# uingei/hevc

Hardware: AMD Instinct MI355X
Metric: encoded 1080p30 frames/sec/GPU; PSNR-Y parity vs libx265 at matched bitrate (higher is better)
Workload: dtype u8; 1 GPU; 1920x1080@30 SDR 8-bit Main, crf 19 capped by VBV maxrate 2940 kbps / bufsize 3528 kbit (the reference's libx265 operating point), 300-frame synthetic 'motion' clip per GPU, keyint 90 (4 closed GOPs of equal length), IPPP, full-search +-15, one clip per GPU, input resident in HBM

## Files before the change

### hevc_amd/_lib.py

```python
from __future__ import annotations

import ctypes as C
import numbers
import os
from pathlib import Path

HERE = Path(__file__).resolve().parent
LIB_PATH = Path(os.environ.get("MIHEVC_LIBRARY", HERE / "libmihevc.so"))

OK, EAGAIN, EOF, EINVAL, ENODEV, ENOMEM, EDEVICE, ESTATE = 0, -1, -2, -3, -4, -5, -6, -7


class Config(C.Structure):
    _fields_ = ([(n, C.c_int32) for n in (
        "width", "height", "fps_num", "fps_den", "bit_depth", "level_idc", "tier", "crf", "qp", "vbv_maxrate_kbps",
        "vbv_bufsize_kbits", "keyint", "min_keyint", "colour_primaries", "transfer", "matrix", "full_range", "chroma_loc",
        "aud", "repeat_headers", "hdr10")] +
        [("md_primaries", (C.c_uint16 * 2) * 3), ("md_white", C.c_uint16 * 2), ("md_max_lum", C.c_uint32), ("md_min_lum", C.c_uint32),
         ("max_cll", C.c_uint16), ("max_fall", C.c_uint16)] +
        [(n, C.c_int32) for n in ("me_range", "gops_in_flight", "host_threads", "sao", "profile_stages", "intra_tiles", "intra_nxn", "intra_in_p", "hrd", "pre_search", "rdo_zero", "chroma_modes", "pic_height", "slice_count", "slice_index")] +
        [("slice_ctu_rows", C.c_int32 * 16), ("rate_share_q16", C.c_int32), ("scenecut", C.c_int32), ("gop_balance", C.c_int32), ("rdo_cg", C.c_int32), ("p_tiles", C.c_int32), ("bframes", C.c_int32), ("b_qp_offset", C.c_int32), ("slice_halo", C.c_int32), ("slice_group", C.c_int32), ("sign_hide", C.c_int32), ("pic_hash", C.c_int32), ("ssim", C.c_int32)])


class Stats(C.Structure):
# ... 170 lines not shown
_PACKED_RGB = {"rgb": (0, 1, 2), "bgr": (2, 1, 0)}


def rgb_format_for(pix_fmt: str, matrix: int = 0, range: int = 0):
    import re
    name = (pix_fmt or "").lower()
    m = re.fullmatch(r"gbrp(?:(9|10|12|14|16)le|(f32le))?", name)
    if m:
        return RgbFormat(0, 2, 0, 1, 2 if m.group(2) else 0, 0 if m.group(2) else int(m.group(1) or 8), matrix, range)
    m = re.fullmatch(r"(rgb|bgr)(24|48le)", name)
    if m:
        return RgbFormat(3, *_PACKED_RGB[m.group(1)], 0, 8 if m.group(2) == "24" else 16, matrix, range)
    m = re.fullmatch(r"(rgb|bgr)(?:[a0]|(a64le))", name)
    if m:
        return RgbFormat(4, *_PACKED_RGB[m.group(1)], 0, 16 if m.group(2) else 8, matrix, range)
    m = re.fullmatch(r"[a0](rgb|bgr)", name)
    if m:
        return RgbFormat(4, *(i + 1 for i in _PACKED_RGB[m.group(1)]), 0, 8, matrix, range)
    return None


EXPORTS = (
    "mihevc_abi_version", "mihevc_device_count", "mihevc_device_numa_node", "mihevc_config_default", "mihevc_open", "mihevc_send_frame", "mihevc_send_frame_async", "mihevc_sync_uploads", "mihevc_send_frame_device", "mihevc_send_frames_device",
    "mihevc_receive_packet", "mihevc_flush", "mihevc_abort", "mihevc_close", "mihevc_get_stats", "mihevc_get_headers", "mihevc_set_keep_recon",
    "mihevc_get_recon", "mihevc_coded_size", "mihevc_get_frame_info", "mihevc_strerror", "mihevc_last_error", "mihevc_cost_params_for_qp", "mihevc_tile_grid", "mihevc_p_tile_grid", "mihevc_k_transform", "mihevc_k_transform_sdh",
    "mihevc_k_intra_frame", "mihevc_k_inter_frame", "mihevc_k_b_frame", "mihevc_k_deblock", "mihevc_k_sao", "mihevc_k_loop_filter", "mihevc_write_parameter_sets",
    "mihevc_encode_picture_host", "mihevc_k_picture_hash", "mihevc_write_picture_hash_sei", "mihevc_get_frame_quality", "mihevc_k_ssim",
    "mihevc_send_frame_fmt", "mihevc_k_convert_source", "mihevc_k_intra_plan", "mihevc_send_frame_rgb", "mihevc_k_convert_rgb",
    "mihevc_send_frame_scaled", "mihevc_k_scale_source", "mihevc_k_scene_diff", "mihevc_send_frame_deint", "mihevc_k_deinterlace",
    "mihevc_send_frame_denoise", "mihevc_k_denoise", "mihevc_send_frame_fieldmatch", "mihevc_get_fieldmatch_info", "mihevc_k_fieldmatch_metrics",
    "mihevc_k_fieldmatch_weave", "mihevc_set_lut3d", "mihevc_send_frame_lut3d", "mihevc_k_lut3d",
    "mihevc_send_frame_interpolate", "mihevc_k_mcfi_vectors", "mihevc_k_mcfi_render",
    "mihevc_send_frame_upscaled", "mihevc_k_upscale_source",
    "mihevc_set_sr_model", "mihevc_send_frame_sr", "mihevc_k_sr_conv", "mihevc_k_sr_input", "mihevc_k_sr_network",
)

_lib = None


class MihevcError(RuntimeError):
    def __init__(self, code: int, what: str = ""):
        self.code = code
        msg = strerror(code)
        super().__init__(f"{what}: {msg} ({code})" if what else f"{msg} ({code})")


def load() -> C.CDLL:
    global _lib
    if _lib is not None:
        return _lib
    if not LIB_PATH.exists():
        raise OSError(f"{LIB_PATH} not built: run `python -c 'import __graft_entry__ as g; g.build()'` (hipcc --offload-arch=gfx950)")
    lib = C.CDLL(str(LIB_PATH))
    for name in EXPORTS:
        getattr(lib, name)
    vp, i32, i64 = C.c_void_p, C.c_int, C.c_int64
    lib.mihevc_strerror.restype = C.c_char_p
    lib.mihevc_last_error.restype = C.c_char_p
    lib.mihevc_last_error.argtypes = [vp]
    lib.mihevc_config_default.argtypes = [C.POINTER(Config)]
    lib.mihevc_config_default.restype = None
    lib.mihevc_open.argtypes = [C.POINTER(Config), i32, C.POINTER(vp)]
    lib.mihevc_send_frame.argtypes = [vp, vp, vp, vp, i32, i32, i64]
    lib.mihevc_send_frame_device.argtypes = [vp, vp, vp, vp, i32, i32, i64]
    lib.mihevc_send_frame_async.argtypes = [vp, vp, vp, vp, i32, i32, i64]
    lib.mihevc_send_frames_device.argtypes = [vp, i32, vp, vp, vp, i32, i32, i64]
    lib.mihevc_sync_uploads.argtypes = [vp]
    lib.mihevc_receive_packet.argtypes = [vp, C.POINTER(C.POINTER(C.c_uint8)), C.POINTER(C.c_size_t), C.POINTER(i64), C.POINTER(i64), C.POINTER(i32)]
    lib.mihevc_flush.argtypes = [vp]
    lib.mihevc_abort.argtypes = [vp]
    lib.mihevc_close.argtypes = [vp]
    lib.mihevc_close.restype = None
    lib.mihevc_get_stats.argtypes = [vp, C.POINTER(Stats)]
    lib.mihevc_get_headers.argtypes = [vp, C.POINTER(C.POINTER(C.c_uint8)), C.POINTER(C.c_size_t)]
    lib.mihevc_set_keep_recon.argtypes = [vp, i32]
    lib.mihevc_get_recon.argtypes = [vp, i64, vp, vp, vp]
    lib.mihevc_coded_size.argtypes = [vp, C.POINTER(i32), C.POINTER(i32)]
    lib.mihevc_get_frame_info.argtypes = [vp, i64, C.POINTER(i32), C.POINTER(i32), C.POINTER(i64)]
    lib.mihevc_cost_params_for_qp.argtypes = [i32, i32, i32, C.POINTER(CostParams)]
    lib.mihevc_cost_params_for_qp.restype = None
    lib.mihevc_k_transform.argtypes = [i32, vp, vp, vp, i32, i32, i32, i32, i32, i32]
    lib.mihevc_k_transform_sdh.argtypes = [i32, vp, vp, vp, i32, i32, i32, i32, i32, i32, i32, i32]
    lib.mihevc_k_intra_frame.argtypes = [i32, vp, vp, vp, i32, i32, C.POINTER(CostParams), vp, vp, vp, vp, vp, vp, vp, vp]
    lib.mihevc_k_intra_plan.argtypes = [i32, vp, vp, vp, i32, i32, C.POINTER(CostParams), vp]
    lib.mihevc_k_inter_frame.argtypes = [i32, vp, vp, vp, vp, vp, vp, i32, i32, C.POINTER(CostParams), vp, vp, vp, vp, vp, vp, vp, vp, vp, vp]
    lib.mihevc_k_b_frame.argtypes = [i32] + [vp] * 9 + [i32, i32, C.POINTER(CostParams)] + [vp] * 12
    lib.mihevc_k_deblock.argtypes = [i32, vp, vp, vp, i32, i32, vp, i32]
    lib.mihevc_k_sao.argtypes = [i32, vp, vp, vp, vp, vp, vp, i32, i32, C.POINTER(CostParams), vp, vp, vp, vp]
    lib.mihevc_k_loop_filter.argtypes = [i32, vp, vp, vp, vp, vp, vp, i32, i32, vp, C.POINTER(CostParams), vp, vp, vp, vp]
    lib.mihevc_write_parameter_sets.argtypes = [C.POINTER(Config), vp, C.c_size_t]
    lib.mihevc_encode_picture_host.argtypes = [C.POINTER(Config), i32, i32, i32, vp, vp, vp, vp, vp, vp, C.c_size_t]
# ... 70 lines not shown
```

### hevc_amd/csrc/bitstream.cpp

```cpp
#include "bitstream.h"

#include <algorithm>
#include <cstdlib>
#include <cstring>

namespace mihevc {

void BitWriter::put(uint32_t v, int n)
{
    while (n > 0) {
        int take = std::min(n, 8 - nbits_);
        uint32_t chunk = (n == 32 && take == 32) ? v : ((v >> (n - take)) & ((1u << take) - 1));
        acc_ = (acc_ << take) | chunk;
        nbits_ += take;
        n -= take;
        if (nbits_ == 8) {
            buf_.push_back((uint8_t)acc_);
            acc_ = 0;
            nbits_ = 0;
        }
    }
}
void BitWriter::ue(uint32_t v)
{
// ... 623 lines not shown
    const TileGrid &grid() const { return grid_; }
    const std::string &error() const { return err_; }
    size_t run_tile(int tx, int ty, std::vector<uint8_t> &out)
    {
        cabac_.redirect(out);
        cabac_.init(pic_.slice_type, pic_.qp);
        const bool last_tile = tx == grid_.cols - 1 && ty == grid_.rows - 1;
        const int x1 = grid_.col_bd(tx + 1), y1 = grid_.row_bd(ty + 1);
        for (int ry = grid_.row_bd(ty); ry < y1; ry++)
            for (int rx = grid_.col_bd(tx); rx < x1; rx++) {
                if (pic_.sao) sao(rx, ry);
                quadtree(rx << kCtuLog2, ry << kCtuLog2, kCtuLog2, 0);
                cabac_.terminate(last_tile && ry == y1 - 1 && rx == x1 - 1);
            }
        if (!last_tile) cabac_.terminate(1);
        cabac_.finish();
        return cabac_.bins();
    }

private:
    const mihevc_cu_rec &cu(int x, int y) const { return pic_.cu[(y >> 3) * w8_ + (x >> 3)]; }
    static int zorder6(int bx, int by)
    {
        int z = 0;
        for (int i = 0; i < 3; i++) z |= ((bx >> i) & 1) << (2 * i) | ((by >> i) & 1) << (2 * i + 1);
        return z;
    }
    int zaddr(int x, int y) const { return (((y >> kCtuLog2) * wc_ + (x >> kCtuLog2)) << 6) | zorder6((x & 31) >> 2, (y & 31) >> 2); }
    bool avail(int xc, int yc, int xn, int yn) const
    {
        if (!(xn >= 0 && yn >= 0 && xn < w_ && yn < h_ && zaddr(xn, yn) <= zaddr(xc, yc))) return false;
        return !grid_.on() || (grid_.col_of(xn >> kCtuLog2) == grid_.col_of(xc >> kCtuLog2) && grid_.row_of(yn >> kCtuLog2) == grid_.row_of(yc >> kCtuLog2));
    }

    void sao(int rx, int ry)
    {
        const mihevc_sao_ctu &s = pic_.sao[ry * wc_ + rx];
        auto same = [](const mihevc_sao_ctu &a, const mihevc_sao_ctu &b) {
            if (a.type[0] != b.type[0] || a.type[1] != b.type[1]) return false;
            for (int c = 0; c < 3; c++) {
                int t = a.type[c ? 1 : 0];
                if (!t) continue;
                if (memcmp(a.offset[c], b.offset[c], 4)) return false;
                if (t == 1 && a.band_pos[c] != b.band_pos[c]) return false;
                if (t == 2 && c < 2 && a.eo_class[c] != b.eo_class[c]) return false;
            }
            return true;
        };
        if (rx > grid_.col_bd(grid_.col_of(rx))) {
// ... 343 lines not shown
                cabac_.bin(kCsbf + ((right | below) ? 1 : 0) + (c_idx ? 2 : 0), 0);
                continue;
            }
            int lev[16], nsig = 0, first_sig = 16, last_sig = -1, abs_sum = 0;
            int start = i == last_sb ? last_pos : 15;
            for (int k = 0; k < 16; k++) {
                lev[k] = k <= start ? b[pscan[k][1] * stride + pscan[k][0]] : 0;
                if (lev[k]) { nsig++; first_sig = std::min(first_sig, k); last_sig = k; abs_sum += std::abs(lev[k]); }
            }
            const bool hidden = sdh && last_sig - first_sig > 3;
            if (hidden && (abs_sum & 1) != (lev[first_sig] < 0) && err_.empty()) {
                const int sh = c_idx ? 1 : 0;
                err_ = "sign data hiding: CTU (" + std::to_string((tu_x << sh) >> kCtuLog2) + ", " + std::to_string((tu_y << sh) >> kCtuLog2) + ") plane " +
                       std::to_string(c_idx) + ": the 4x4 group at (" + std::to_string(tu_x + 4 * xs) + ", " + std::to_string(tu_y + 4 * ys) +
                       ") has an absolute sum whose parity does not match its first level's sign";
            }
            bool infer_dc = false;
            if (i < last_sb && i > 0) {
                csbf[ys][xs] = nsig != 0;
                cabac_.bin(kCsbf + ((right | below) ? 1 : 0) + (c_idx ? 2 : 0), nsig != 0);
                infer_dc = true;
            } else csbf[ys][xs] = 1;
            if (!csbf[ys][xs]) continue;
            int prev = right + 2 * below;
            for (int k = (i == last_sb ? last_pos - 1 : 15); k >= 0; k--) {
                if (k == 0 && infer_dc) break;
                int xp = pscan[k][0], yp = pscan[k][1], xc = (xs << 2) + xp, yc = (ys << 2) + yp, sc;
                if (log2n == 2) { static const uint8_t m[16] = {0, 1, 4, 5, 2, 3, 4, 5, 6, 6, 8, 8, 7, 7, 8, 8}; sc = m[(yc << 2) + xc]; }
                else if (xc + yc == 0) sc = 0;
                else {
                    if (prev == 0) sc = (xp + yp == 0) ? 2 : (xp + yp < 3) ? 1 : 0;
                    else if (prev == 1) sc = yp == 0 ? 2 : yp == 1 ? 1 : 0;
                    else if (prev == 2) sc = xp == 0 ? 2 : xp == 1 ? 1 : 0;
                    else sc = 2;
                    if (c_idx == 0) { if (xs || ys) sc += 3; sc += log2n == 3 ? (scan == 0 ? 9 : 15) : 21; }
                    else sc += log2n == 3 ? 9 : 12;
                }
                cabac_.bin(kSig + (c_idx ? 27 + sc : sc), lev[k] != 0);
                if (lev[k]) infer_dc = false;
            }
            if (!nsig) continue;
            int ctx_set = (i > 0 && c_idx == 0) ? 2 : 0;
            if (c1_carry == 0) ctx_set++;
            int c1 = 1, ng1 = 0, g2_pos = -1;
            for (int k = 15; k >= 0; k--) {
                if (!lev[k]) continue;
                if (ng1 == 8) break;
                int g1 = std::abs(lev[k]) > 1;
                cabac_.bin(kG1 + ctx_set * 4 + c1 + (c_idx ? 16 : 0), g1);
                ng1++;
                if (g1) { c1 = 0; if (g2_pos < 0) g2_pos = k; }
                else if (c1 > 0 && c1 < 3) c1++;
            }
            c1_carry = c1;
            if (g2_pos >= 0) cabac_.bin(kG2 + ctx_set + (c_idx ? 4 : 0), std::abs(lev[g2_pos]) > 2);
            uint32_t signs = 0; int ns = 0;
            for (int k = 15; k >= 0; k--) if (lev[k]) { signs = (signs << 1) | (uint32_t)(lev[k] < 0); ns++; }
            if (hidden) { signs >>= 1; ns--; }
            cabac_.bypass_bits(signs, ns);
            int num = 0, rice = 0;
            for (int k = 15; k >= 0; k--) {
                if (!lev[k]) continue;
                int a = std::abs(lev[k]);
                int base = num < 8 ? (k == g2_pos ? 3 : 2) : 1;
                if (a >= base) {
                    remaining(a - base, rice);
                    if (a > 3 * (1 << rice)) rice = std::min(rice + 1, 4);
                }
                num++;
            }
        }
    }
    void remaining(int v, int rice)
    {
        int q = v >> rice;
        if (q < 4) {
            for (int i = 0; i < q; i++) cabac_.bypass(1);
            cabac_.bypass(0);
            cabac_.bypass_bits((uint32_t)(v & ((1 << rice) - 1)), rice);
        } else {
            for (int i = 0; i < 4; i++) cabac_.bypass(1);
            int k = rice + 1, r = v - (4 << rice);
            while (r >= (1 << k)) { cabac_.bypass(1); r -= 1 << k; k++; }
            cabac_.bypass(0);
            cabac_.bypass_bits((uint32_t)r, k);
        }
    }

    const mihevc_config &cfg_;
    const PictureSyms &pic_;
    std::vector<uint8_t> scratch_;
    Cabac cabac_;
// ... 108 lines not shown
```

### hevc_amd/csrc/session.cpp

```cpp
#include <algorithm>
#include <chrono>
#include <cstdlib>
#include <cstring>
#include <numeric>
#include <thread>

#include "md5.h"
#include "session.h"

constexpr int kSeamRows = 8;

int fail(mihevc_session *s, std::string msg)
{
    { std::lock_guard<std::mutex> l(s->m); s->err = std::move(msg); }
    s->failed = true;
    if (s->group) s->group->fail();
    return MIHEVC_EDEVICE;
}

int alloc_planes(mihevc_session *s, CachedBlock<uint8_t> mem[3], void *p[3], int stride[3], int padded)
{
    for (int i = 0; i < 3; i++) {
        int w = i ? s->w / 2 : s->w, h = i ? s->h / 2 : s->h, pad = padded == 1 ? (i ? PAD_C : PAD_Y) : 0, vm = padded == 2 ? (i ? kSeamRows / 2 : kSeamRows) : pad;
        stride[i] = (w + 2 * pad + 63) & ~63;
// ... 563 lines not shown

template <typename T> std::vector<FrameRec> lane_records(mihevc_session *s, const Chunk<T> &c, int g, int upto)
{
    std::vector<FrameRec> v((size_t)upto);
    std::lock_guard<std::mutex> l(s->m);
    for (int j = 0; j < upto; j++) v[(size_t)j] = s->frames[c.fidx(g, j)];
    return v;
}

int slice_sums(mihevc_session *s, const std::vector<size_t> &idx, bool with_est)
{
    const size_t n = idx.size();
    std::vector<double> v(with_est ? 2 * n : n);
    {
        std::lock_guard<std::mutex> l(s->m);
        for (size_t i = 0; i < n; i++) { v[i] = (double)s->frames[idx[i]].bits_local; if (with_est) v[n + i] = (double)s->frames[idx[i]].est_local; }
    }
    if (int e = group_sum(s, v)) return e;
    std::lock_guard<std::mutex> l(s->m);
    for (size_t i = 0; i < n; i++) { auto &fr = s->frames[idx[i]]; fr.bits = (long long)v[i]; if (with_est) { fr.est_q4 = (unsigned long long)v[n + i]; fr.est_known = true; } }
    return 0;
}

int lane_estimates(mihevc_session *s, const SymLayout &sl, int slot, const std::vector<int> &lanes, std::vector<unsigned long long> &out)
{
    std::vector<double> v(lanes.size(), 0.0);
    for (size_t k = 0; k < lanes.size(); k++) {
        unsigned long long e = 0;
        HIPCK(s, hipMemcpy(&e, s->lane[lanes[k]].sym_dev[slot] + sl.est, sizeof e, hipMemcpyDeviceToHost));
        v[k] = (double)e;
    }
    if (int e = group_sum(s, v)) return e;
    out.assign(v.begin(), v.end());
    return 0;
}
std::vector<int> first_lanes(int n) { std::vector<int> v((size_t)n); std::iota(v.begin(), v.end(), 0); return v; }

int mark(mihevc_session *s, hipStream_t st, int stage, int pictures, bool begin)
{
    if (!s->cfg.profile_stages || (s->cfg.profile_stages == 2 && stage != 2)) return 0;
    size_t need_ev = s->marks.size() * 2 + 2;
    while (s->ev_pool.size() < need_ev) { s->ev_pool.emplace_back(hipEventDefault); if (!s->ev_pool.back()) return fail(s, "hipEventCreate failed"); }
    if (begin) { s->marks.push_back({stage, pictures, s->marks.size() * 2}); HIPCK(s, hipEventRecord(s->ev_pool[s->marks.back().ev], st)); }
    else HIPCK(s, hipEventRecord(s->ev_pool[s->marks.back().ev + 1], st));
    return 0;
}
#define STAGE(st, idx, pics, call) do { if (int e_ = mark(s, st, idx, pics, true)) return e_; HIPCK(s, call); if (int e_ = mark(s, st, idx, pics, false)) return e_; } while (0)

template <typename T> int rate_feedback(mihevc_session *s, const Chunk<T> &c, const Part &p, int t)
{
    const int p_slots = s->ring - 1;
    if (c.halo.on && s->rc.rc_on && t - p_slots >= 1) {
        std::vector<size_t> idx;
        for (int g = 0; g < c.gl.batch[(size_t)(t - p_slots)]; g++) idx.push_back(c.fidx(g, t - p_slots));
        if (int e = slice_sums(s, idx, false)) return e;
    }
    if (t >= 2) HIPCK(s, hipStreamWaitEvent(p.st, s->slot[t == 2 ? 0 : p.grp][c.slot_of(t - 2)].copy, 0));
    if (!s->rc.rc_on || t < 3) return 0;
    const int j = t - 2;
    const Part pj = c.part(s, p.grp, j);
    HIPCK(s, hipEventSynchronize(s->slot[p.grp][c.slot_of(j)].copy));
    std::vector<double> v((size_t)pj.n);
    for (int k = 0; k < pj.n; k++) v[(size_t)k] = (double)*(const unsigned long long *)(s->lane[pj.lanes[(size_t)k]].sym_host[c.slot_of(j)] + c.sl.est);
    if (int e = group_sum(s, v)) return e;
    std::lock_guard<std::mutex> l(s->m);
    for (int k = 0; k < pj.n; k++) { auto &fr = s->frames[c.fidx(pj.lanes[(size_t)k], j)]; if (!fr.est_known) { fr.est_q4 = (unsigned long long)v[(size_t)k]; fr.est_known = true; } }
    return 0;
}

template <typename T> int rho_trial(mihevc_session *s, const Chunk<T> &c, const std::vector<int> &want, const std::vector<unsigned long long> &ev, const std::vector<int> &qa)
{
    const int B1 = c.gl.batch[1], tb = c.steps;
    memcpy(c.ha + (size_t)tb * c.lay.total, c.ha + (size_t)1 * c.lay.total, c.lay.total);
    StepView<T> tv(c.ha, c.lay, tb), dtv(c.da, c.lay, tb), h0(c.ha, c.lay, 0), h1(c.ha, c.lay, 1);
    std::vector<int> qp_trial((size_t)B1);
    for (int g = 0; g < B1; g++) {
        mihevc_session::Lane &L = s->lane[g];
        const int a = c.at(1, g);
        qp_trial[(size_t)g] = RateControl::trial_qp(want[(size_t)g]);
        tv.sao[a] = h0.sao[c.at(0, g)];
        tv.sao[a].sao = nullptr; tv.sao[a].sse = nullptr; tv.sao[a].sse_ctu = nullptr; tv.sao[a].cu = nullptr;
        tv.sao[a].halo_top = tv.sao[a].halo_bottom = 0;
        tv.inter[a] = h1.inter[a];
        for (int i = 0; i < 3; i++) tv.inter[a].rec[i] = mk<T>(L.rec_p[1][i], L.rec_stride[i]);
        tv.inter[a].prm = prm_for(s, qp_trial[(size_t)g]);
        tv.inter[a].ip = nullptr;
        HIPCK(s, hipMemsetAsync(L.sym_dev[c.slot_of(1)] + c.sl.sse, 0, 4 * sizeof(unsigned long long), s->st_compute));
    }
    HIPCK(s, hipMemcpyAsync(c.da + (size_t)tb * c.lay.total, c.ha + (size_t)tb * c.lay.total, c.lay.total, hipMemcpyHostToDevice, s->st_compute));
    HIPCK(s, launch_sao<T>(s->st_compute, dtv.sao, s->w, s->h, B1, false));
    HIPCK(s, launch_pad<T>(s->st_compute, dtv.sao, s->w, s->h, B1));
    if (s->cfg.pre_search) HIPCK(s, hipStreamWaitEvent(s->st_compute, s->ev_pre, 0));
    HIPCK(s, launch_me_search<T>(s->st_compute, dtv.inter, s->n_ctu, B1, s->me_range));
    HIPCK(s, launch_inter_ctu<T>(s->st_compute, dtv.inter, s->n_ctu, B1, s->me_range));
    HIPCK(s, hipStreamSynchronize(s->st_compute));
    std::vector<unsigned long long> ep;
    if (int e = lane_estimates(s, c.sl, c.slot_of(1), first_lanes(B1), ep)) return e;
    s->rc.measure_rho(ep, qp_trial, ev, qa);
    return 0;
}

template <typename T> int idr_step(mihevc_session *s, const Chunk<T> &c, std::vector<int> &qp_step)
{
    const int B = c.gl.batch[0];
    StepView<T> dv(c.da, c.lay, 0), hv(c.ha, c.lay, 0);
    HIPCK(s, hipMemcpyAsync(c.da, c.ha, c.lay.total, hipMemcpyHostToDevice, s->st_compute));
    for (int g = 0; g < B; g++) HIPCK(s, hipMemsetAsync(s->lane[g].sym_dev[0] + c.sl.sse, 0, 4 * sizeof(unsigned long long), s->st_compute));
    STAGE(s->st_compute, 0, B, launch_intra_picture<T>(s->st_compute, dv.intra, s->ctus_w, s->ctus_h, B, s->tiles.cols, s->tiles.rows, s->cfg.pre_search ? s->ev_args : nullptr));
    if (s->cfg.pre_search) {
        HIPCK(s, hipStreamWaitEvent(s->st_pre, s->ev_args, 0));
        HIPCK(s, launch_pre_search_chunk<T>(s->st_pre, (const PreArgs<T> *)(c.da + c.flat_off), s->w, s->h, s->n_ctu, c.n_pre));
        HIPCK(s, hipEventRecord(s->ev_pre, s->st_pre));
    }
    if (!s->rc.rc_on) return 0;
    HIPCK(s, hipStreamSynchronize(s->st_compute));
    std::vector<unsigned long long> ev, e2;
    if (int e = lane_estimates(s, c.sl, 0, first_lanes(B), ev)) return e;
    const std::vector<int> qa(qp_step);
    std::vector<int> want((size_t)B);
    for (int g = 0; g < B; g++) want[(size_t)g] = s->rc.want_idr(g, ev[(size_t)g], qa[(size_t)g]);
    if (!s->rc.rho_measured && c.steps > 1 && c.gl.batch[1] > 0) {
        if (int e = rho_trial<T>(s, c, want, ev, qa)) return e;
        for (int g = 0; g < B; g++) want[(size_t)g] = s->rc.want_idr(g, ev[(size_t)g], qa[(size_t)g]);
    }
    std::vector<int> redo;
    for (int g = 0; g < B; g++)
        if (RateControl::redo_idr(want[(size_t)g], qa[(size_t)g])) redo.push_back(g);
    if (!redo.empty()) {
        for (size_t k = 0; k < redo.size(); k++) {
            const int g = redo[k];
            qp_step[(size_t)g] = want[(size_t)g];
            patch_qp<T>(s, c, 0, g, qp_step[(size_t)g]);
            hv.intra[B + (int)k] = hv.intra[c.at(0, g)];
            HIPCK(s, hipMemsetAsync(s->lane[g].sym_dev[0] + c.sl.sse, 0, 4 * sizeof(unsigned long long), s->st_compute));
        }
        HIPCK(s, hipMemcpyAsync(c.da, c.ha, c.lay.total, hipMemcpyHostToDevice, s->st_compute));
        STAGE(s->st_compute, 0, (int)redo.size(), launch_intra_picture<T>(s->st_compute, dv.intra + B, s->ctus_w, s->ctus_h, (int)redo.size(), s->tiles.cols, s->tiles.rows, nullptr));
        HIPCK(s, hipStreamSynchronize(s->st_compute));
        if (int e = lane_estimates(s, c.sl, 0, redo, e2)) return e;
        for (size_t k = 0; k < redo.size(); k++) ev[(size_t)redo[k]] = e2[k];
    }
    s->rc.idr_settled(qp_step);
    std::lock_guard<std::mutex> l(s->m);
    for (int g = 0; g < B; g++) { auto &fr = s->frames[c.fidx(g, 0)]; fr.est_q4 = ev[(size_t)g]; fr.est_known = true; }
    return 0;
}

template <typename T> int inter_step(mihevc_session *s, const Chunk<T> &c, const Part &p, int t)
{
    const int B = p.n;
    hipStream_t st = p.st;
    StepView<T> dv(c.da, c.lay, t, p.base), hv(c.ha, c.lay, t, p.base), pv(c.da, c.lay, t - 1, c.group_base(p.grp, t - 1));
    StepParams sp{};
    sp.p_tile_cols = s->ptiles.cols; sp.p_tile_rows = s->ptiles.rows;
    for (int g = 0; g < B; g++) sp.prm[g] = hv.inter[g].prm;
    if (c.halo.on && c.halo.reach > 0) {
        if (int e = wait_neighbours(s, c.halo, 2, s->gstep + t - 1)) return e;
        HIPCK(s, launch_copy_rows(st, c.halo.jobs(t, c.halo.jl.pull), B * 3 * c.halo.reach, 16));
    }
    HIPCK(s, launch_prep_p_step<T>(st, pv.sao, (const PreArgs<T> *)nullptr, dv.intra, dv.inter, dv.sao, sp, s->w, s->h, B));
    if (t == 1 && s->cfg.pre_search) HIPCK(s, hipStreamWaitEvent(st, s->ev_pre, 0));
    const bool bstep = type_of_step(c.bf, t) == 0;
// ... 329 lines not shown
{
    if (!s) return MIHEVC_EINVAL;
    if (s->failed) return s->fail_code;
    if (s->flushed) return MIHEVC_OK;
    if (int e = source_flush(s)) return e;
    s->flushing = true;
    int e = run_chunk(s);
    s->flushed = true;
    return e;
}

int mihevc_abort(mihevc_session *s)
{
    if (!s) return MIHEVC_EINVAL;
    { std::lock_guard<std::mutex> l(s->m); if (s->err.empty()) s->err = "aborted by the caller"; }
    s->failed = true;
    if (s->group) s->group->fail();
    return MIHEVC_OK;
}

int mihevc_receive_packet(mihevc_session *s, const uint8_t **data, size_t *size, int64_t *pts, int64_t *dts, int *keyframe)
{
    if (!s || !data || !size) return MIHEVC_EINVAL;
    std::unique_lock<std::mutex> l(s->m);
    auto it = s->packets.find(s->next_out);
    if (it == s->packets.end() || !it->second.ready) return (s->flushed && s->next_out >= s->frames_in) ? MIHEVC_EOF : MIHEVC_EAGAIN;
    if (!it->second.error.empty()) { std::string err = it->second.error; l.unlock(); s->fail_code = MIHEVC_EINVAL; fail(s, err); return MIHEVC_EINVAL; }
    s->cur_packet = std::move(it->second.data);
    if (pts) *pts = it->second.pts;
    if (dts) *dts = it->second.dts;
    if (keyframe) *keyframe = it->second.key;
    s->packets.erase(it);
    s->next_out++;
    s->stats.frames_out = s->next_out;
    *data = s->cur_packet.data();
    *size = s->cur_packet.size();
    return MIHEVC_OK;
}

int mihevc_get_headers(mihevc_session *s, const uint8_t **data, size_t *size)
{
    if (!s || !data || !size) return MIHEVC_EINVAL;
    *data = s->headers.data();
    *size = s->headers.size();
    return MIHEVC_OK;
}

int mihevc_get_stats(const mihevc_session *s, mihevc_stats *out)
{
    if (!s || !out) return MIHEVC_EINVAL;
    std::lock_guard<std::mutex> l(const_cast<mihevc_session *>(s)->m);
    *out = s->stats;
    out->entropy_ms = (double)s->entropy_ns.load() / 1e6;
    double *ssim[3] = {&out->ssim_y, &out->ssim_u, &out->ssim_v};
    for (int c = 0; c < 3; c++) *ssim[c] = s->cfg.ssim ? (double)s->ssim_total[c] / ((double)ssim_window_count(s, c) * 4294967296.0) : 0.0;
    return MIHEVC_OK;
}

int mihevc_set_keep_recon(mihevc_session *s, int keep)
{
    if (!s) return MIHEVC_EINVAL;
    s->keep_recon = keep != 0;
// ... 66 lines not shown
```

### hevc_amd/csrc/session.h

```cpp
#pragma once
#include <hip/hip_runtime.h>

#include <atomic>
#include <condition_variable>
#include <map>
#include <mutex>
#include <string>
#include <vector>

#include "bitstream.h"
#include "device.h"
#include "gop_plan.h"
#include "host_pool.h"
#include "ratectl.h"
#include "scale_taps.h"
#include "slice_group.h"

using namespace mihevc;

constexpr int kRing = 12;
constexpr int kGroups = 2;

struct Packet {
    std::vector<uint8_t> data;
// ... 42 lines not shown
    int keyint = 90, lanes = 4, me_range = 16, qp_p = 22, qp_i = 19;
    bool is16 = false, keep_recon = false, flushed = false, flushing = false;
    std::atomic<bool> failed{false};
    int fail_code = MIHEVC_EDEVICE;
    std::string err;
    CachedStream st_compute, st_copy, st_pre;
    int lane_groups = kGroups;
    Event ev_up{hipEventDisableTiming};
    bool up_pending = false;
    std::vector<Src> pending;
    std::vector<Src> free_src;
    SourceFront src;
    struct Lane {
        CachedBlock<uint8_t> rec_mem[3][3]; void *rec_p[3][3] = {}; int rec_stride[3] = {};
        CachedBlock<uint8_t> work_mem[3]; void *work_p[3] = {}; int work_stride[3] = {};
        CachedBlock<int32_t> me, me1;
        CachedBlock<IpInfo> ip;
        CachedBlock<IntraPlan> plan;
        CachedBlock<uint8_t> sym_dev[kRing], sym_host[kRing];
        CachedBlock<uint8_t> md5_host[kRing];
    };
    std::vector<Lane> lane;
    CachedBuf args;
    struct Slot { Event compute{hipEventDisableTiming}, copy{hipEventDisableTiming}; int jobs_open = 0; } slot[kGroups][kRing];
    Event ev_join{hipEventDisableTiming};
    Event t_begin{hipEventDefault}, t_end{hipEventDefault};
    std::vector<Event> ev_pool;
    struct Mark { int stage, pictures; size_t ev; };
    std::vector<Mark> marks;
    ThreadPool *pool = nullptr;
    std::mutex m;
    std::condition_variable cv;
    int ring = 8;
    int host_threads = 2;
    std::map<int64_t, Packet> packets;
    int64_t next_out = 0, frames_in = 0, frames_done = 0;
    std::vector<uint8_t> headers, cur_packet;
    std::map<int64_t, std::vector<uint16_t>> recon;
    mihevc_stats stats{};
    RateControl rc;
    CachedBuf probe;
    int64_t pts_step = 1, first_pts = 0;
    GopState gop;
    CachedBuf low;
    Event ev_pre{hipEventDisableTiming}, ev_args{hipEventDisableTiming};
    CachedBuf scene;
    std::vector<FrameRec> frames;
    struct Quality { unsigned long long sse[3]; long long ssim[3]; bool known; };
    std::vector<Quality> quality;
    std::atomic<long long> entropy_ns{0};
    bool events_ok() const
    {
        bool ok = ev_up && ev_join && t_begin && t_end && ev_pre && ev_args;
        for (auto &g : slot) for (auto &sl : g) ok = ok && sl.compute && sl.copy;
        return ok;
    }
    std::shared_ptr<SliceGroup> group;
    int band = 0, n_bands = 1;
    int band_h[kMaxBands] = {0};
    long long gstep = 0;
// ... 21 lines not shown
```

### hevc_amd/encoder.py

```python
from __future__ import annotations

import ctypes as C
import logging
import re
import threading
from fractions import Fraction
from pathlib import Path
from typing import Callable, Iterator, Optional, Tuple

import numpy as np

from . import _lib
from .probe import VideoInfo

logger = logging.getLogger(__name__)

_COLOUR_CODES = {
    "primaries": {"bt709": 1, "bt470bg": 5, "smpte170m": 6, "bt2020": 9},
    "transfer": {"bt709": 1, "smpte170m": 6, "smpte2084": 16, "pq": 16, "arib-std-b67": 18, "bt2020-10": 14},
    "matrix": {"bt709": 1, "bt470bg": 5, "smpte170m": 6, "bt2020nc": 9, "bt2020-ncl": 9, "bt2020": 9},
}


_DEPTH_IN_FMT = re.compile(r'(?:p|gray|gbrp|yuva?\d{3}p?)(9|10|12|14|16)(?:le|be)?$|^(?:p0|p2|p4|y2)(10|12|16)(?:le|be)?$')
# ... 38 lines not shown
            cfg.md_primaries[i][0], cfg.md_primaries[i][1] = x, y
        cfg.md_white[0], cfg.md_white[1] = md.wp
        cfg.md_max_lum, cfg.md_min_lum = md.lum
        cfg.max_cll, cfg.max_fall = parse_max_cll(max_cll or info.max_cll)
    else:
        cfg.colour_primaries = _COLOUR_CODES["primaries"].get(info.color_primaries, 1)
        cfg.transfer = _COLOUR_CODES["transfer"].get(info.color_transfer, 1)
        cfg.matrix = _COLOUR_CODES["matrix"].get(info.color_space, 1)
    return cfg


class Encoder:

    def __init__(self, cfg: _lib.Config, device: int = 0, keep_recon: bool = False):
        self._lib = _lib.load()
        self.cfg = cfg
        self._s = C.c_void_p()
        rc = self._lib.mihevc_open(C.byref(cfg), device, C.byref(self._s))
        if rc != 0:
            raise _lib.MihevcError(rc, "mihevc_open")
        if keep_recon:
            self._lib.mihevc_set_keep_recon(self._s, 1)
        self._pts = 0

    def close(self):
        if self._s:
            self._lib.mihevc_close(self._s)
            self._s = C.c_void_p()

    def __enter__(self):
        return self

    def __exit__(self, *exc):
        self.close()

    def _check(self, rc, what):
        if rc != 0:
            detail = self._lib.mihevc_last_error(self._s).decode() if self._s else ""
            raise _lib.MihevcError(rc, f"{what} {detail}".strip())

    def send(self, y: np.ndarray, u: np.ndarray, v: np.ndarray, pts: Optional[int] = None):
        c = self.cfg
        dt = np.uint8 if c.bit_depth == 8 else np.uint16
        if y.shape != (c.height, c.width) or u.shape != (c.height // 2, c.width // 2) or v.shape != u.shape:
            raise ValueError(f"plane shapes {y.shape}/{u.shape}/{v.shape} do not match the session's {c.width}x{c.height} 4:2:0")
        for p in (y, u, v):
# ... 249 lines not shown

    def sync_uploads(self):
        self._check(self._lib.mihevc_sync_uploads(self._s), "sync_uploads")

    def send_device(self, y_ptr: int, u_ptr: int, v_ptr: int, pitch_y: int, pitch_c: int, pts: Optional[int] = None):
        pts = self._pts if pts is None else pts
        self._pts = pts + 1
        self._check(self._lib.mihevc_send_frame_device(self._s, y_ptr, u_ptr, v_ptr, pitch_y, pitch_c, pts), "send_frame_device")

    def send_device_batch(self, y_ptrs, u_ptrs, v_ptrs, pitch_y: int, pitch_c: int, first_pts: Optional[int] = None):
        n = len(y_ptrs)
        arrs = [p if isinstance(p, C.Array) else (C.c_void_p * n)(*p) for p in (y_ptrs, u_ptrs, v_ptrs)]
        pts = self._pts if first_pts is None else first_pts
        self._pts = pts + n
        self._check(self._lib.mihevc_send_frames_device(self._s, n, arrs[0], arrs[1], arrs[2], pitch_y, pitch_c, pts), "send_frames_device")

    def flush(self):
        self._check(self._lib.mihevc_flush(self._s), "flush")

    def abort(self):
        if self._s:
            self._lib.mihevc_abort(self._s)

    def packets(self) -> Iterator[Tuple[bytes, int, bool]]:
        data, size = C.POINTER(C.c_uint8)(), C.c_size_t()
        pts, dts, key = C.c_int64(), C.c_int64(), C.c_int()
        while True:
            rc = self._lib.mihevc_receive_packet(self._s, C.byref(data), C.byref(size), C.byref(pts), C.byref(dts), C.byref(key))
            if rc in (_lib.EAGAIN, _lib.EOF):
                return
            self._check(rc, "receive_packet")
            yield C.string_at(data, size.value), pts.value, bool(key.value)

    def packets_dts(self) -> Iterator[Tuple[bytes, int, bool, int]]:
        data, size = C.POINTER(C.c_uint8)(), C.c_size_t()
        pts, dts, key = C.c_int64(), C.c_int64(), C.c_int()
        while True:
            rc = self._lib.mihevc_receive_packet(self._s, C.byref(data), C.byref(size), C.byref(pts), C.byref(dts), C.byref(key))
            if rc in (_lib.EAGAIN, _lib.EOF):
                return
            self._check(rc, "receive_packet")
            yield C.string_at(data, size.value), pts.value, bool(key.value), dts.value

    def headers(self) -> bytes:
        data, size = C.POINTER(C.c_uint8)(), C.c_size_t()
        self._check(self._lib.mihevc_get_headers(self._s, C.byref(data), C.byref(size)), "get_headers")
        return C.string_at(data, size.value)

    def stats(self) -> _lib.Stats:
        st = _lib.Stats()
        self._check(self._lib.mihevc_get_stats(self._s, C.byref(st)), "get_stats")
        return st

    def coded_size(self) -> Tuple[int, int]:
        w, h = C.c_int(), C.c_int()
        self._lib.mihevc_coded_size(self._s, C.byref(w), C.byref(h))
        return w.value, h.value

    def recon(self, index: int):
        w, h = self.coded_size()
        y, u, v = np.zeros((h, w), np.uint16), np.zeros((h // 2, w // 2), np.uint16), np.zeros((h // 2, w // 2), np.uint16)
        self._check(self._lib.mihevc_get_recon(self._s, index, y.ctypes.data, u.ctypes.data, v.ctypes.data), "get_recon")
        return y, u, v

    def frame_info(self, index: int):
# ... 572 lines not shown
```

### include/mihevc.h

```cpp
#ifndef MIHEVC_H
#define MIHEVC_H
#include <stddef.h>
#include <stdint.h>

#ifdef __cplusplus
extern "C" {
#endif

#define MIHEVC_ABI_VERSION 6

typedef enum {
    MIHEVC_OK = 0,
    MIHEVC_EAGAIN = -1,
    MIHEVC_EOF = -2,
    MIHEVC_EINVAL = -3,
    MIHEVC_ENODEV = -4,
    MIHEVC_ENOMEM = -5,
    MIHEVC_EDEVICE = -6,
    MIHEVC_ESTATE = -7
} mihevc_err;

typedef struct mihevc_config {
    int32_t width, height;
    int32_t fps_num, fps_den;
// ... 152 lines not shown
    int32_t reserved[5];
} mihevc_interpolate;
int  mihevc_send_frame_interpolate(mihevc_session *s, const mihevc_interpolate *d, const void *y, const void *u, const void *v,
                                   int pitch_y, int pitch_c, int64_t pts, int flags);
typedef struct mihevc_upscale_src {
    int32_t width, height;
    int32_t bit_depth;
    int32_t sharpen;
    int32_t antiring;
    int32_t reserved[3];
} mihevc_upscale_src;
int  mihevc_send_frame_upscaled(mihevc_session *s, const mihevc_upscale_src *src, const void *y, const void *u, const void *v,
                                int pitch_y, int pitch_c, int64_t pts, int flags);
typedef struct mihevc_sr_model {
    int32_t scale;
    int32_t blocks;
    int32_t reserved[6];
} mihevc_sr_model;
int  mihevc_set_sr_model(mihevc_session *s, const mihevc_sr_model *model, const float *weights, size_t count);
int  mihevc_send_frame_sr(mihevc_session *s, const mihevc_rgb_format *fmt, int src_width, int src_height, const void *p0, const void *p1, const void *p2,
                          int pitch, int64_t pts, int flags);
int  mihevc_receive_packet(mihevc_session *s, const uint8_t **data, size_t *size,
                           int64_t *pts, int64_t *dts, int *keyframe);
int  mihevc_flush(mihevc_session *s);
int  mihevc_abort(mihevc_session *s);
void mihevc_close(mihevc_session *s);
int  mihevc_get_stats(const mihevc_session *s, mihevc_stats *out);
int  mihevc_get_headers(mihevc_session *s, const uint8_t **data, size_t *size);
int  mihevc_set_keep_recon(mihevc_session *s, int keep);
int  mihevc_get_recon(mihevc_session *s, int64_t index, uint16_t *y, uint16_t *u, uint16_t *v);
int  mihevc_coded_size(const mihevc_session *s, int *w, int *h);
int  mihevc_get_frame_info(mihevc_session *s, int64_t index, int *qp, int *slice_type, int64_t *bits);
int  mihevc_get_frame_quality(mihevc_session *s, int64_t index, uint64_t sse[3], int64_t ssim_q32[3], int64_t ssim_windows[3]);
const char *mihevc_strerror(int err);
const char *mihevc_last_error(const mihevc_session *s);

typedef struct mihevc_cost_params {
    int32_t qp, qp_c, bit_depth, lambda_sad_q4, lambda_q4, me_range;
    int32_t tile_cols, tile_rows;
    int32_t intra_nxn;
    int32_t intra_in_p;
    int32_t pre_search;
    int32_t rdo_zero;
    int32_t chroma_modes;
    int32_t mc_top, mc_bottom;
    int32_t rdo_cg;
// ... 116 lines not shown
```

Before: 6279 frames/s.

## Batch packet retrieval, async rate-control estimate readback, and streamline CABAC residual coding

Adds a batched receive_packets API so Python drains up to 512 packets per ctypes call instead of one. Replaces the per-lane synchronous hipMemcpy of rate-control estimates with async copies into pinned host memory and a single stream sync, and overlaps rho-trial host preparation with the IDR intra kernels. Also simplifies CABAC significance-context derivation with precomputed pattern tables and a gathered absolute-level array, plus a table-based z-order. These target host-side latency and per-call overhead, at the cost of extra API surface and per-batch packet storage.

New measurement: 6458 frames/s, median of 6. 2.8% higher.

```diff
diff --git a/hevc_amd/_lib.py b/hevc_amd/_lib.py
--- a/hevc_amd/_lib.py
+++ b/hevc_amd/_lib.py
@@ -216,7 +216,7 @@
 
 EXPORTS = (
     "mihevc_abi_version", "mihevc_device_count", "mihevc_device_numa_node", "mihevc_config_default", "mihevc_open", "mihevc_send_frame", "mihevc_send_frame_async", "mihevc_sync_uploads", "mihevc_send_frame_device", "mihevc_send_frames_device",
-    "mihevc_receive_packet", "mihevc_flush", "mihevc_abort", "mihevc_close", "mihevc_get_stats", "mihevc_get_headers", "mihevc_set_keep_recon",
+    "mihevc_receive_packet", "mihevc_receive_packets", "mihevc_flush", "mihevc_abort", "mihevc_close", "mihevc_get_stats", "mihevc_get_headers", "mihevc_set_keep_recon",
     "mihevc_get_recon", "mihevc_coded_size", "mihevc_get_frame_info", "mihevc_strerror", "mihevc_last_error", "mihevc_cost_params_for_qp", "mihevc_tile_grid", "mihevc_p_tile_grid", "mihevc_k_transform", "mihevc_k_transform_sdh",
     "mihevc_k_intra_frame", "mihevc_k_inter_frame", "mihevc_k_b_frame", "mihevc_k_deblock", "mihevc_k_sao", "mihevc_k_loop_filter", "mihevc_write_parameter_sets",
     "mihevc_encode_picture_host", "mihevc_k_picture_hash", "mihevc_write_picture_hash_sei", "mihevc_get_frame_quality", "mihevc_k_ssim",
@@ -261,6 +261,7 @@
     lib.mihevc_send_frames_device.argtypes = [vp, i32, vp, vp, vp, i32, i32, i64]
     lib.mihevc_sync_uploads.argtypes = [vp]
     lib.mihevc_receive_packet.argtypes = [vp, C.POINTER(C.POINTER(C.c_uint8)), C.POINTER(C.c_size_t), C.POINTER(i64), C.POINTER(i64), C.POINTER(i32)]
+    lib.mihevc_receive_packets.argtypes = [vp, i32, vp, vp, vp, vp, vp]
     lib.mihevc_flush.argtypes = [vp]
     lib.mihevc_abort.argtypes = [vp]
     lib.mihevc_close.argtypes = [vp]
diff --git a/hevc_amd/csrc/bitstream.cpp b/hevc_amd/csrc/bitstream.cpp
--- a/hevc_amd/csrc/bitstream.cpp
+++ b/hevc_amd/csrc/bitstream.cpp
@@ -669,9 +669,8 @@
     const mihevc_cu_rec &cu(int x, int y) const { return pic_.cu[(y >> 3) * w8_ + (x >> 3)]; }
     static int zorder6(int bx, int by)
     {
-        int z = 0;
-        for (int i = 0; i < 3; i++) z |= ((bx >> i) & 1) << (2 * i) | ((by >> i) & 1) << (2 * i + 1);
-        return z;
+        static const uint8_t spread[8] = {0, 1, 4, 5, 16, 17, 20, 21};
+        return spread[bx] | (spread[by] << 1);
     }
     int zaddr(int x, int y) const { return (((y >> kCtuLog2) * wc_ + (x >> kCtuLog2)) << 6) | zorder6((x & 31) >> 2, (y & 31) >> 2); }
     bool avail(int xc, int yc, int xn, int yn) const
@@ -1061,52 +1060,45 @@
                 infer_dc = true;
             } else csbf[ys][xs] = 1;
             if (!csbf[ys][xs]) continue;
-            int prev = right + 2 * below;
+            static const uint8_t pat[5][16] = {
+                {0, 1, 4, 5, 2, 3, 4, 5, 6, 6, 8, 8, 7, 7, 8, 8},
+                {2, 1, 1, 0, 1, 1, 0, 0, 1, 0, 0, 0, 0, 0, 0, 0},
+                {2, 2, 2, 2, 1, 1, 1, 1, 0, 0, 0, 0, 0, 0, 0, 0},
+                {2, 1, 0, 0, 2, 1, 0, 0, 2, 1, 0, 0, 2, 1, 0, 0},
+                {2, 2, 2, 2, 2, 2, 2, 2, 2, 2, 2, 2, 2, 2, 2, 2}};
+            const uint8_t *sig_pat = pat[log2n == 2 ? 0 : 1 + right + 2 * below];
+            const int sig_off = kSig + (c_idx ? 27 : 0) +
+                                (log2n == 2 ? 0 : c_idx == 0 ? ((xs || ys) ? 3 : 0) + (log2n == 3 ? (scan == 0 ? 9 : 15) : 21) : (log2n == 3 ? 9 : 12));
             for (int k = (i == last_sb ? last_pos - 1 : 15); k >= 0; k--) {
                 if (k == 0 && infer_dc) break;
-                int xp = pscan[k][0], yp = pscan[k][1], xc = (xs << 2) + xp, yc = (ys << 2) + yp, sc;
-                if (log2n == 2) { static const uint8_t m[16] = {0, 1, 4, 5, 2, 3, 4, 5, 6, 6, 8, 8, 7, 7, 8, 8}; sc = m[(yc << 2) + xc]; }
-                else if (xc + yc == 0) sc = 0;
-                else {
-                    if (prev == 0) sc = (xp + yp == 0) ? 2 : (xp + yp < 3) ? 1 : 0;
-                    else if (prev == 1) sc = yp == 0 ? 2 : yp == 1 ? 1 : 0;
-                    else if (prev == 2) sc = xp == 0 ? 2 : xp == 1 ? 1 : 0;
-                    else sc = 2;
-                    if (c_idx == 0) { if (xs || ys) sc += 3; sc += log2n == 3 ? (scan == 0 ? 9 : 15) : 21; }
-                    else sc += log2n == 3 ? 9 : 12;
-                }
-                cabac_.bin(kSig + (c_idx ? 27 + sc : sc), lev[k] != 0);
+                const int ctx = (k == 0 && i == 0 && log2n != 2) ? kSig + (c_idx ? 27 : 0) : sig_off + sig_pat[(pscan[k][1] << 2) | pscan[k][0]];
+                cabac_.bin(ctx, lev[k] != 0);
                 if (lev[k]) infer_dc = false;
             }
             if (!nsig) continue;
             int ctx_set = (i > 0 && c_idx == 0) ? 2 : 0;
             if (c1_carry == 0) ctx_set++;
-            int c1 = 1, ng1 = 0, g2_pos = -1;
-            for (int k = 15; k >= 0; k--) {
-                if (!lev[k]) continue;
-                if (ng1 == 8) break;
-                int g1 = std::abs(lev[k]) > 1;
+            int av[16], ns = 0;
+            uint32_t signs = 0;
+            for (int k = 15; k >= 0; k--) if (lev[k]) { av[ns++] = std::abs(lev[k]); signs = (signs << 1) | (uint32_t)(lev[k] < 0); }
+            int c1 = 1, g2_at = -1;
+            for (int j = 0; j < ns && j < 8; j++) {
+                int g1 = av[j] > 1;
                 cabac_.bin(kG1 + ctx_set * 4 + c1 + (c_idx ? 16 : 0), g1);
-                ng1++;
-                if (g1) { c1 = 0; if (g2_pos < 0) g2_pos = k; }
+                if (g1) { c1 = 0; if (g2_at < 0) g2_at = j; }
                 else if (c1 > 0 && c1 < 3) c1++;
             }
             c1_carry = c1;
-            if (g2_pos >= 0) cabac_.bin(kG2 + ctx_set + (c_idx ? 4 : 0), std::abs(lev[g2_pos]) > 2);
-            uint32_t signs = 0; int ns = 0;
-            for (int k = 15; k >= 0; k--) if (lev[k]) { signs = (signs << 1) | (uint32_t)(lev[k] < 0); ns++; }
-            if (hidden) { signs >>= 1; ns--; }
-            cabac_.bypass_bits(signs, ns);
-            int num = 0, rice = 0;
-            for (int k = 15; k >= 0; k--) {
-                if (!lev[k]) continue;
-                int a = std::abs(lev[k]);
-                int base = num < 8 ? (k == g2_pos ? 3 : 2) : 1;
+            if (g2_at >= 0) cabac_.bin(kG2 + ctx_set + (c_idx ? 4 : 0), av[g2_at] > 2);
+            if (hidden) cabac_.bypass_bits(signs >> 1, ns - 1);
+            else cabac_.bypass_bits(signs, ns);
+            int rice = 0;
+            for (int j = 0; j < ns; j++) {
+                const int a = av[j], base = j < 8 ? (j == g2_at ? 3 : 2) : 1;
                 if (a >= base) {
                     remaining(a - base, rice);
                     if (a > 3 * (1 << rice)) rice = std::min(rice + 1, 4);
                 }
-                num++;
             }
         }
     }
diff --git a/hevc_amd/csrc/session.cpp b/hevc_amd/csrc/session.cpp
--- a/hevc_amd/csrc/session.cpp
+++ b/hevc_amd/csrc/session.cpp
@@ -609,14 +609,18 @@
     return 0;
 }
 
-int lane_estimates(mihevc_session *s, const SymLayout &sl, int slot, const std::vector<int> &lanes, std::vector<unsigned long long> &out)
-{
-    std::vector<double> v(lanes.size(), 0.0);
-    for (size_t k = 0; k < lanes.size(); k++) {
-        unsigned long long e = 0;
-        HIPCK(s, hipMemcpy(&e, s->lane[lanes[k]].sym_dev[slot] + sl.est, sizeof e, hipMemcpyDeviceToHost));
-        v[k] = (double)e;
-    }
+int queue_estimates(mihevc_session *s, const SymLayout &sl, int slot, const std::vector<int> &lanes)
+{
+    if (!s->est_host) HIPCK(s, s->est_host.alloc(s->device, MAX_LANES * sizeof(unsigned long long), true));
+    for (size_t k = 0; k < lanes.size(); k++)
+        HIPCK(s, hipMemcpyAsync(s->est_host + k, s->lane[lanes[k]].sym_dev[slot] + sl.est, sizeof(unsigned long long), hipMemcpyDeviceToHost, s->st_compute));
+    return 0;
+}
+int wait_estimates(mihevc_session *s, size_t n, std::vector<unsigned long long> &out)
+{
+    HIPCK(s, hipStreamSynchronize(s->st_compute));
+    std::vector<double> v(n, 0.0);
+    for (size_t k = 0; k < n; k++) v[k] = (double)s->est_host[k];
     if (int e = group_sum(s, v)) return e;
     out.assign(v.begin(), v.end());
     return 0;
@@ -655,24 +659,32 @@
     return 0;
 }
 
-template <typename T> int rho_trial(mihevc_session *s, const Chunk<T> &c, const std::vector<int> &want, const std::vector<unsigned long long> &ev, const std::vector<int> &qa)
+template <typename T> int rho_trial_prepare(mihevc_session *s, const Chunk<T> &c)
 {
     const int B1 = c.gl.batch[1], tb = c.steps;
     memcpy(c.ha + (size_t)tb * c.lay.total, c.ha + (size_t)1 * c.lay.total, c.lay.total);
-    StepView<T> tv(c.ha, c.lay, tb), dtv(c.da, c.lay, tb), h0(c.ha, c.lay, 0), h1(c.ha, c.lay, 1);
-    std::vector<int> qp_trial((size_t)B1);
+    StepView<T> tv(c.ha, c.lay, tb), h0(c.ha, c.lay, 0), h1(c.ha, c.lay, 1);
     for (int g = 0; g < B1; g++) {
         mihevc_session::Lane &L = s->lane[g];
         const int a = c.at(1, g);
-        qp_trial[(size_t)g] = RateControl::trial_qp(want[(size_t)g]);
         tv.sao[a] = h0.sao[c.at(0, g)];
         tv.sao[a].sao = nullptr; tv.sao[a].sse = nullptr; tv.sao[a].sse_ctu = nullptr; tv.sao[a].cu = nullptr;
         tv.sao[a].halo_top = tv.sao[a].halo_bottom = 0;
         tv.inter[a] = h1.inter[a];
         for (int i = 0; i < 3; i++) tv.inter[a].rec[i] = mk<T>(L.rec_p[1][i], L.rec_stride[i]);
-        tv.inter[a].prm = prm_for(s, qp_trial[(size_t)g]);
         tv.inter[a].ip = nullptr;
         HIPCK(s, hipMemsetAsync(L.sym_dev[c.slot_of(1)] + c.sl.sse, 0, 4 * sizeof(unsigned long long), s->st_compute));
+    }
+    return 0;
+}
+template <typename T> int rho_trial(mihevc_session *s, const Chunk<T> &c, const std::vector<int> &want, const std::vector<unsigned long long> &ev, const std::vector<int> &qa)
+{
+    const int B1 = c.gl.batch[1], tb = c.steps;
+    StepView<T> tv(c.ha, c.lay, tb), dtv(c.da, c.lay, tb);
+    std::vector<int> qp_trial((size_t)B1);
+    for (int g = 0; g < B1; g++) {
+        qp_trial[(size_t)g] = RateControl::trial_qp(want[(size_t)g]);
+        tv.inter[c.at(1, g)].prm = prm_for(s, qp_trial[(size_t)g]);
     }
     HIPCK(s, hipMemcpyAsync(c.da + (size_t)tb * c.lay.total, c.ha + (size_t)tb * c.lay.total, c.lay.total, hipMemcpyHostToDevice, s->st_compute));
     HIPCK(s, launch_sao<T>(s->st_compute, dtv.sao, s->w, s->h, B1, false));
@@ -680,9 +692,9 @@
     if (s->cfg.pre_search) HIPCK(s, hipStreamWaitEvent(s->st_compute, s->ev_pre, 0));
     HIPCK(s, launch_me_search<T>(s->st_compute, dtv.inter, s->n_ctu, B1, s->me_range));
     HIPCK(s, launch_inter_ctu<T>(s->st_compute, dtv.inter, s->n_ctu, B1, s->me_range));
-    HIPCK(s, hipStreamSynchronize(s->st_compute));
+    if (int e = queue_estimates(s, c.sl, c.slot_of(1), first_lanes(B1))) return e;
     std::vector<unsigned long long> ep;
-    if (int e = lane_estimates(s, c.sl, c.slot_of(1), first_lanes(B1), ep)) return e;
+    if (int e = wait_estimates(s, (size_t)B1, ep)) return e;
     s->rc.measure_rho(ep, qp_trial, ev, qa);
     return 0;
 }
@@ -694,19 +706,21 @@
     HIPCK(s, hipMemcpyAsync(c.da, c.ha, c.lay.total, hipMemcpyHostToDevice, s->st_compute));
     for (int g = 0; g < B; g++) HIPCK(s, hipMemsetAsync(s->lane[g].sym_dev[0] + c.sl.sse, 0, 4 * sizeof(unsigned long long), s->st_compute));
     STAGE(s->st_compute, 0, B, launch_intra_picture<T>(s->st_compute, dv.intra, s->ctus_w, s->ctus_h, B, s->tiles.cols, s->tiles.rows, s->cfg.pre_search ? s->ev_args : nullptr));
+    if (s->rc.rc_on) { if (int e = queue_estimates(s, c.sl, 0, first_lanes(B))) return e; }
     if (s->cfg.pre_search) {
         HIPCK(s, hipStreamWaitEvent(s->st_pre, s->ev_args, 0));
         HIPCK(s, launch_pre_search_chunk<T>(s->st_pre, (const PreArgs<T> *)(c.da + c.flat_off), s->w, s->h, s->n_ctu, c.n_pre));
         HIPCK(s, hipEventRecord(s->ev_pre, s->st_pre));
     }
     if (!s->rc.rc_on) return 0;
-    HIPCK(s, hipStreamSynchronize(s->st_compute));
+    const bool trial = !s->rc.rho_measured && c.steps > 1 && c.gl.batch[1] > 0;
+    if (trial) { if (int e = rho_trial_prepare<T>(s, c)) return e; }
     std::vector<unsigned long long> ev, e2;
-    if (int e = lane_estimates(s, c.sl, 0, first_lanes(B), ev)) return e;
+    if (int e = wait_estimates(s, (size_t)B, ev)) return e;
     const std::vector<int> qa(qp_step);
     std::vector<int> want((size_t)B);
     for (int g = 0; g < B; g++) want[(size_t)g] = s->rc.want_idr(g, ev[(size_t)g], qa[(size_t)g]);
-    if (!s->rc.rho_measured && c.steps > 1 && c.gl.batch[1] > 0) {
+    if (trial) {
         if (int e = rho_trial<T>(s, c, want, ev, qa)) return e;
         for (int g = 0; g < B; g++) want[(size_t)g] = s->rc.want_idr(g, ev[(size_t)g], qa[(size_t)g]);
     }
@@ -723,8 +737,8 @@
         }
         HIPCK(s, hipMemcpyAsync(c.da, c.ha, c.lay.total, hipMemcpyHostToDevice, s->st_compute));
         STAGE(s->st_compute, 0, (int)redo.size(), launch_intra_picture<T>(s->st_compute, dv.intra + B, s->ctus_w, s->ctus_h, (int)redo.size(), s->tiles.cols, s->tiles.rows, nullptr));
-        HIPCK(s, hipStreamSynchronize(s->st_compute));
-        if (int e = lane_estimates(s, c.sl, 0, redo, e2)) return e;
+        if (int e = queue_estimates(s, c.sl, 0, redo)) return e;
+        if (int e = wait_estimates(s, redo.size(), e2)) return e;
         for (size_t k = 0; k < redo.size(); k++) ev[(size_t)redo[k]] = e2[k];
     }
     s->rc.idr_settled(qp_step);
@@ -1100,6 +1114,7 @@
 int mihevc_receive_packet(mihevc_session *s, const uint8_t **data, size_t *size, int64_t *pts, int64_t *dts, int *keyframe)
 {
     if (!s || !data || !size) return MIHEVC_EINVAL;
+    s->cur_batch.clear();
     std::unique_lock<std::mutex> l(s->m);
     auto it = s->packets.find(s->next_out);
     if (it == s->packets.end() || !it->second.ready) return (s->flushed && s->next_out >= s->frames_in) ? MIHEVC_EOF : MIHEVC_EAGAIN;
@@ -1116,6 +1131,33 @@
     return MIHEVC_OK;
 }
 
+int mihevc_receive_packets(mihevc_session *s, int max, const uint8_t **data, size_t *size, int64_t *pts, int64_t *dts, int *keyframe)
+{
+    if (!s || max <= 0 || !data || !size) return MIHEVC_EINVAL;
+    s->cur_batch.clear();
+    std::unique_lock<std::mutex> l(s->m);
+    int n = 0;
+    auto it = s->packets.find(s->next_out);
+    while (n < max && it != s->packets.end() && it->first == s->next_out && it->second.ready) {
+        if (!it->second.error.empty()) {
+            if (n) break;
+            std::string err = it->second.error; l.unlock(); s->fail_code = MIHEVC_EINVAL; fail(s, err); return MIHEVC_EINVAL;
+        }
+        s->cur_batch.push_back(std::move(it->second.data));
+        data[n] = s->cur_batch.back().data();
+        size[n] = s->cur_batch.back().size();
+        if (pts) pts[n] = it->second.pts;
+        if (dts) dts[n] = it->second.dts;
+        if (keyframe) keyframe[n] = it->second.key;
+        it = s->packets.erase(it);
+        s->next_out++;
+        n++;
+    }
+    if (!n) return (s->flushed && s->next_out >= s->frames_in) ? MIHEVC_EOF : MIHEVC_EAGAIN;
+    s->stats.frames_out = s->next_out;
+    return n;
+}
+
 int mihevc_get_headers(mihevc_session *s, const uint8_t **data, size_t *size)
 {
     if (!s || !data || !size) return MIHEVC_EINVAL;
diff --git a/hevc_amd/csrc/session.h b/hevc_amd/csrc/session.h
--- a/hevc_amd/csrc/session.h
+++ b/hevc_amd/csrc/session.h
@@ -88,6 +88,7 @@
     };
     std::vector<Lane> lane;
     CachedBuf args;
+    CachedBlock<unsigned long long> est_host;
     struct Slot { Event compute{hipEventDisableTiming}, copy{hipEventDisableTiming}; int jobs_open = 0; } slot[kGroups][kRing];
     Event ev_join{hipEventDisableTiming};
     Event t_begin{hipEventDefault}, t_end{hipEventDefault};
@@ -102,6 +103,7 @@
     std::map<int64_t, Packet> packets;
     int64_t next_out = 0, frames_in = 0, frames_done = 0;
     std::vector<uint8_t> headers, cur_packet;
+    std::vector<std::vector<uint8_t>> cur_batch;
     std::map<int64_t, std::vector<uint16_t>> recon;
     mihevc_stats stats{};
     RateControl rc;
diff --git a/hevc_amd/encoder.py b/hevc_amd/encoder.py
--- a/hevc_amd/encoder.py
+++ b/hevc_amd/encoder.py
@@ -84,6 +84,8 @@
         if keep_recon:
             self._lib.mihevc_set_keep_recon(self._s, 1)
         self._pts = 0
+        self._arrays = None
+        self._ready = []
 
     def close(self):
         if self._s:
@@ -379,25 +381,29 @@
         if self._s:
             self._lib.mihevc_abort(self._s)
 
+    _BATCH = 512
+
+    def _receive_batch(self) -> bool:
+        if self._arrays is None:
+            n = self._BATCH
+            self._arrays = ((C.c_void_p * n)(), (C.c_size_t * n)(), (C.c_int64 * n)(), (C.c_int64 * n)(), (C.c_int * n)())
+        data, size, pts, dts, key = self._arrays
+        n = self._lib.mihevc_receive_packets(self._s, self._BATCH, data, size, pts, dts, key)
+        if n in (_lib.EAGAIN, _lib.EOF):
+            return False
+        if n < 0:
+            self._check(n, "receive_packets")
+        at = C.string_at
+        self._ready = [(at(d, s), p, k != 0, t) for d, s, p, k, t in zip(data[:n], size[:n], pts[:n], key[:n], dts[:n])][::-1]
+        return True
+
     def packets(self) -> Iterator[Tuple[bytes, int, bool]]:
-        data, size = C.POINTER(C.c_uint8)(), C.c_size_t()
-        pts, dts, key = C.c_int64(), C.c_int64(), C.c_int()
-        while True:
-            rc = self._lib.mihevc_receive_packet(self._s, C.byref(data), C.byref(size), C.byref(pts), C.byref(dts), C.byref(key))
-            if rc in (_lib.EAGAIN, _lib.EOF):
-                return
-            self._check(rc, "receive_packet")
-            yield C.string_at(data, size.value), pts.value, bool(key.value)
+        while self._ready or self._receive_batch():
+            yield self._ready.pop()[:3]
 
     def packets_dts(self) -> Iterator[Tuple[bytes, int, bool, int]]:
-        data, size = C.POINTER(C.c_uint8)(), C.c_size_t()
-        pts, dts, key = C.c_int64(), C.c_int64(), C.c_int()
-        while True:
-            rc = self._lib.mihevc_receive_packet(self._s, C.byref(data), C.byref(size), C.byref(pts), C.byref(dts), C.byref(key))
-            if rc in (_lib.EAGAIN, _lib.EOF):
-                return
-            self._check(rc, "receive_packet")
-            yield C.string_at(data, size.value), pts.value, bool(key.value), dts.value
+        while self._ready or self._receive_batch():
+            yield self._ready.pop()
 
     def headers(self) -> bytes:
         data, size = C.POINTER(C.c_uint8)(), C.c_size_t()
diff --git a/include/mihevc.h b/include/mihevc.h
--- a/include/mihevc.h
+++ b/include/mihevc.h
@@ -198,6 +198,8 @@
                           int pitch, int64_t pts, int flags);
 int  mihevc_receive_packet(mihevc_session *s, const uint8_t **data, size_t *size,
                            int64_t *pts, int64_t *dts, int *keyframe);
+int  mihevc_receive_packets(mihevc_session *s, int max, const uint8_t **data, size_t *size,
+                            int64_t *pts, int64_t *dts, int *keyframe);
 int  mihevc_flush(mihevc_session *s);
 int  mihevc_abort(mihevc_session *s);
 void mihevc_close(mihevc_session *s);
```
